# VictoriaMetrics/VictoriaMetrics

Hardware: NVIDIA H100
Metric: rollup samples/sec (block decode + rate, raw samples decoded and scanned per second) (higher is better)
Workload: dtype int64 codec -> f64 rollup

## Files before the change

victoriametrics_b200/csrc/api.cu:

```cuda
#include <cuda_runtime.h>
#include <cuda_fp16.h>
#include <stdarg.h>
#include <stdio.h>
#include <string.h>
#include <stdlib.h>

#include <algorithm>
#include <vector>

#include "common.cuh"
#include "decode.cu"
#include "rollup.cu"
#include "fused.cu"
#include "zstd.cu"
#include "marshal.inc"
#include "encode.cu"

static thread_local char g_err[512];
void vmb_set_error(const char* fmt, ...) {
    va_list ap;
    va_start(ap, fmt);
    vsnprintf(g_err, sizeof(g_err), fmt, ap);
    va_end(ap);
}
// ... 167 lines not shown
    vmb_ctx_comm_destroy(c);
    if (c->col_cache) vmb_series_free(c->col_cache);
    c->col_cache = nullptr;
    DevBuf* bufs[] = {&c->zscratch, &c->zlit, &c->zstatus, &c->zjobs, &c->zws, &c->args1, &c->args2, &c->rolled,
                      &c->counters, &c->tmp_out, &c->grp, &c->mheap, &c->mnext, &c->zseq, &c->bail, &c->sub_arrays, &c->fused_recs, &c->aggr_state, &c->grp_ids, &c->enc_vals, &c->enc_deltas, &c->enc_out, &c->enc_meta, &c->enc_frames,
                      &c->oa_keys, &c->oa_keys2, &c->oa_cell, &c->oa_meta, &c->cv_runs, &c->cv_aux, &c->cv_uniq};
    for (DevBuf* b : bufs) b->release();
    for (cudaEvent_t e : c->ev)
        if (e) cudaEventDestroy(e);
    for (cudaEvent_t e : c->zev) cudaEventDestroy(e);
    if (c->zstream) cudaStreamDestroy(c->zstream);
    if (c->h_pinned) cudaFreeHost(c->h_pinned);
    if (c->pipe && c->pipe_destroy) c->pipe_destroy(c->pipe);
    delete c;
}
extern "C" int vmb_ctx_set_stream(vmb_ctx* c, void* stream) {
    if (!c) return VMB_ERR_INVALID_ARG;
    c->stream = (cudaStream_t)stream;
    return VMB_OK;
}
extern "C" int vmb_ctx_set_dedup_interval(vmb_ctx* c, int64_t interval_ms) {
    if (!c || interval_ms < 0) return VMB_ERR_INVALID_ARG;
    c->dedup_interval = interval_ms;
    return VMB_OK;
}
extern "C" int vmb_ctx_set_fused(vmb_ctx* c, int enable) {
    if (!c) return VMB_ERR_INVALID_ARG;
    c->fused = enable != 0;
    return VMB_OK;
}
extern "C" int vmb_ctx_synchronize(vmb_ctx* c) {
    if (!c) return VMB_ERR_INVALID_ARG;
    CU(cudaSetDevice(c->device));
    CU(cudaStreamSynchronize(c->stream));
    return VMB_OK;
}
extern "C" uint64_t vmb_ctx_launch_count(const vmb_ctx* c) { return c ? c->launches : 0; }
extern "C" float vmb_ctx_last_stage_ms(const vmb_ctx* c, int stage) {
    return (c && stage >= 0 && stage < ST__COUNT) ? c->stage_ms[stage] : 0.f;
}
extern "C" int vmb_ctx_enable_stage_timing(vmb_ctx* c, int enable) {
    if (!c) return VMB_ERR_INVALID_ARG;
    c->timing = enable != 0;
    return VMB_OK;
}
extern "C" void* vmb_host_alloc(size_t bytes) {
    void* p = nullptr;
    if (cudaHostAlloc(&p, bytes ? bytes : 1, cudaHostAllocDefault) != cudaSuccess) return nullptr;
    return p;
}
extern "C" void vmb_host_free(void* p) {
    if (p) cudaFreeHost(p);
}

static inline uint64_t be_get(const uint8_t* s, int n) {
    uint64_t v = 0;
    for (int i = 0; i < n; i++) v = (v << 8) | s[i];
    return v;
}
extern "C" int vmb_block_desc_from_header(vmb_block_desc* d, const uint8_t h[81], uint8_t tsid_out[24]) {
    if (!d || !h) return VMB_ERR_INVALID_ARG;
    memset(d, 0, sizeof(*d));
    if (tsid_out) memcpy(tsid_out, h, 24);
    auto unzz = [](uint64_t u) { return (int64_t)(u >> 1) ^ -(int64_t)(u & 1); };
    d->min_ts = unzz(be_get(h + 24, 8));
    d->max_ts = unzz(be_get(h + 32, 8));
    d->first_value = unzz(be_get(h + 40, 8));
    d->ts_off = be_get(h + 48, 8);
    d->val_off = be_get(h + 56, 8);
    d->ts_size = (uint32_t)be_get(h + 64, 4);
    d->val_size = (uint32_t)be_get(h + 68, 4);
    d->rows = (uint32_t)be_get(h + 72, 4);
    uint16_t u = (uint16_t)be_get(h + 76, 2);
    d->scale = (int16_t)((int16_t)(u >> 1) ^ (int16_t)(-(int16_t)(u & 1)));
    d->ts_mt = h[78];
    d->val_mt = h[79];
    d->precision_bits = h[80];
    if (d->rows == 0 || d->rows > 16384) return VMB_ERR_ROWS;
    if (d->ts_mt > 6 || d->val_mt > 6) return VMB_ERR_MARSHAL_TYPE;
    if (d->precision_bits < 1 || d->precision_bits > 64) return VMB_ERR_INVALID_ARG;
    if (d->ts_size > 131072 || d->val_size > 131072) return VMB_ERR_INVALID_ARG;
    return VMB_OK;
}

static inline void be_put(uint8_t* d, uint64_t v, int n) {
    for (int i = 0; i < n; i++) d[i] = (uint8_t)(v >> (8 * (n - 1 - i)));
}
extern "C" int vmb_block_header_marshal(uint8_t h[81], const vmb_block_desc* d, const uint8_t tsid[24]) {
    if (!h || !d) return VMB_ERR_INVALID_ARG;
    if (tsid) memcpy(h, tsid, 24);
    else memset(h, 0, 24);
    auto zz = [](int64_t v) { return (uint64_t)((v << 1) ^ (v >> 63)); };
    be_put(h + 24, zz(d->min_ts), 8);
    be_put(h + 32, zz(d->max_ts), 8);
    be_put(h + 40, zz(d->first_value), 8);
    be_put(h + 48, d->ts_off, 8);
    be_put(h + 56, d->val_off, 8);
    be_put(h + 64, d->ts_size, 4);
    be_put(h + 68, d->val_size, 4);
    be_put(h + 72, d->rows, 4);
    be_put(h + 76, (uint16_t)((d->scale << 1) ^ (d->scale >> 15)), 2);
    h[78] = d->ts_mt;
    h[79] = d->val_mt;
    h[80] = d->precision_bits;
    return VMB_OK;
}
extern "C" int vmb_index_block_unmarshal(vmb_block_desc* out, uint8_t* tsids, size_t count, const uint8_t* data, size_t len) {
    if (!out || !data || count == 0) return VMB_ERR_INVALID_ARG;
    if (len != count * 81) {
        vmb_set_error("invalid number of block headers found: %zu bytes; want %zu block headers", len, count);
        return len % 81 ? VMB_ERR_SHORT_SRC : VMB_ERR_ROWS;
    }
    for (size_t i = 0; i < count; i++) {
        int rc = vmb_block_desc_from_header(&out[i], data + i * 81, tsids ? tsids + i * 24 : nullptr);
        if (rc) {
            vmb_set_error("cannot unmarshal block header %zu: error %d", i, rc);
            return rc;
        }
        if (i && memcmp(data + (i - 1) * 81, data + i * 81, 24) > 0) {
            vmb_set_error("block headers must be sorted by tsid (header %zu)", i);
            return VMB_ERR_INVALID_ARG;
        }
    }
    return VMB_OK;
}
extern "C" int vmb_metaindex_rows_unmarshal(vmb_metaindex_row* out, size_t cap, size_t* n_out, const uint8_t* data, size_t len) {
    if (!n_out || (len && !data)) return VMB_ERR_INVALID_ARG;
    *n_out = 0;
    if (len == 0) {
        vmb_set_error("expecting non-zero metaindex rows; got zero");
        return VMB_ERR_SHORT_SRC;
    }
    if (len % 56) {
        vmb_set_error("cannot unmarshal metaindexRow #%zu: %zu trailing bytes", len / 56, len % 56);
        return VMB_ERR_SHORT_SRC;
    }
    const size_t n = len / 56;
    *n_out = n;
    if (n > cap || !out) return VMB_ERR_CAP;
    auto unzz = [](uint64_t u) { return (int64_t)(u >> 1) ^ -(int64_t)(u & 1); };
    for (size_t i = 0; i < n; i++) {
        const uint8_t* r = data + i * 56;
        vmb_metaindex_row& m = out[i];
        memcpy(m.tsid, r, 24);
        m.block_headers_count = (uint32_t)be_get(r + 24, 4);
        m.min_ts = unzz(be_get(r + 28, 8));
        m.max_ts = unzz(be_get(r + 36, 8));
        m.index_block_offset = be_get(r + 44, 8);
        m.index_block_size = (uint32_t)be_get(r + 52, 4);
        if (m.block_headers_count == 0) {
            vmb_set_error("metaindexRow #%zu: BlockHeadersCount must be greater than 0", i);
            return VMB_ERR_ROWS;
        }
        if (m.index_block_size > 131072) {
            vmb_set_error("metaindexRow #%zu: too big IndexBlockSize %u", i, m.index_block_size);
            return VMB_ERR_INVALID_ARG;
        }
        if (i && memcmp(r - 56, r, 24) > 0) {
            vmb_set_error("metaindexRow values must be sorted by TSID (row %zu)", i);
            return VMB_ERR_INVALID_ARG;
        }
    }
    return VMB_OK;
}
extern "C" int vmb_metaindex_row_marshal(uint8_t out[56], const vmb_metaindex_row* m) {
    if (!out || !m) return VMB_ERR_INVALID_ARG;
    auto zz = [](int64_t v) { return (uint64_t)((v << 1) ^ (v >> 63)); };
    memcpy(out, m->tsid, 24);
    be_put(out + 24, m->block_headers_count, 4);
    be_put(out + 28, zz(m->min_ts), 8);
    be_put(out + 36, zz(m->max_ts), 8);
    be_put(out + 44, m->index_block_offset, 8);
    be_put(out + 52, m->index_block_size, 4);
    return VMB_OK;
}

template <class T>
static int dev_alloc(T** p, size_t n) {
    *p = nullptr;
    cudaError_t e = cudaMalloc((void**)p, (n ? n : 1) * sizeof(T));
    if (e != cudaSuccess) {
        vmb_set_error("cudaMalloc(%zu) failed: %s", n * sizeof(T), cudaGetErrorString(e));
        return VMB_ERR_NOMEM;
    }
    return 0;
}

extern "C" void vmb_blocks_free(vmb_blocks* b) {
    if (!b) return;
    if (b->ctx) cudaSetDevice(b->ctx->device);
    cudaFree(b->d_arrays);
    cudaFree(b->d_payload_alloc);
    delete b;
}
extern "C" size_t vmb_blocks_count(const vmb_blocks* b) { return b ? b->nblocks : 0; }
extern "C" uint64_t vmb_blocks_rows(const vmb_blocks* b) { return b ? b->rows : 0; }
extern "C" uint64_t vmb_blocks_compressed_bytes(const vmb_blocks* b) { return b ? b->compressed : 0; }

struct BlocksPlan {
    std::vector<ColInfo> cols;
    std::vector<uint64_t> row_off;
    std::vector<uint32_t> huf, gen, bad, ser_first, ser_nblocks, fused, unfused, huf_upto;
    std::vector<uint64_t> ser_merge_off;
    uint64_t rows = 0, compressed = 0, scratch_total = 0, merge_rows = 0, seq_total = 0;
    bool needs_lit = false;
    unsigned long long content_bound = 0;
};
static void plan_layout(BlocksPlan& pl, const vmb_block_desc* descs, size_t nblocks) {
    pl.row_off.resize(nblocks + 1);
    pl.rows = 0;
    pl.ser_first.clear();
    pl.ser_nblocks.clear();
    for (size_t b = 0; b < nblocks; b++) {
        const vmb_block_desc& d = descs[b];
        pl.row_off[b] = pl.rows;
        pl.rows += d.rows <= 16384 ? d.rows : 0;
        if (b == 0 || d.series_idx != descs[b - 1].series_idx) {
            pl.ser_first.push_back((uint32_t)b);
            pl.ser_nblocks.push_back(1);
        } else {
            pl.ser_nblocks.back()++;
        }
    }
    pl.row_off[nblocks] = pl.rows;
    pl.ser_merge_off.assign(pl.ser_first.size(), UINT64_MAX);
    pl.merge_rows = 0;
    std::vector<uint32_t> order;
    for (size_t s = 0; s < pl.ser_first.size(); s++) {
        const uint32_t fb = pl.ser_first[s], nb = pl.ser_nblocks[s];
        if (nb < 2) continue;
        order.resize(nb);
        for (uint32_t k = 0; k < nb; k++) order[k] = fb + k;
        std::stable_sort(order.begin(), order.end(), [&](uint32_t a, uint32_t b) { return descs[a].min_ts < descs[b].min_ts; });
        uint64_t r = pl.row_off[fb], total = 0;
        bool overlap = false;
        for (uint32_t k = 0; k < nb; k++) {
            const vmb_block_desc& d = descs[order[k]];
            const uint64_t rows = d.rows <= 16384 ? d.rows : 0;
            pl.row_off[order[k]] = r + total;
            total += rows;
            if (k + 1 < nb && d.max_ts >= descs[order[k + 1]].min_ts) overlap = true;
        }
        if (overlap) {
            pl.ser_merge_off[s] = pl.merge_rows;
            pl.merge_rows += total;
        }
    }
}

static int plan_blocks(BlocksPlan& pl, const vmb_block_desc* descs, size_t nblocks, const uint8_t* payload, size_t payload_len) {
    pl.cols.resize(2 * nblocks);
    uint64_t scratch = 0;
    for (size_t b = 0; b < nblocks; b++) {
        const vmb_block_desc& d = descs[b];
        pl.compressed += (uint64_t)d.ts_size + d.val_size;
        if ((uint64_t)d.ts_off + d.ts_size > payload_len || (uint64_t)d.val_off + d.val_size > payload_len) {
            vmb_set_error("block %zu: payload range outside the arena (len %zu)", b, payload_len);
            return VMB_ERR_INVALID_ARG;
        }
        for (int which = 0; which < 2; which++) {
            ColInfo& ci = pl.cols[2 * b + which];
            memset(&ci, 0, sizeof(ci));
            int mt = which ? d.val_mt : d.ts_mt;
            if (mt != 1 && mt != 4) continue;
            const uint8_t* src = payload + (which ? d.val_off : d.ts_off);
            uint32_t len = which ? d.val_size : d.ts_size;
            uint32_t cs = 0;
            bool needs_lit = false;
            uint32_t nseq = 0;
            ci.kind = zstd_classify_host(src, len, d.rows <= 16384 ? d.rows : 0, &cs, &needs_lit, &nseq, pl.content_bound);
            if (ci.kind == VMB_ZK_HUF && nseq) {
                if (pl.seq_total + nseq > 0xffffffffull) {
                    vmb_set_error("more than 2^32 zstd sequences in one batch: split it");
                    return VMB_ERR_INVALID_ARG;
                }
                ci.nseq = nseq;
                ci.seq_rec_off = (uint32_t)pl.seq_total;
                pl.seq_total += nseq;
            }
            ci.content_size = cs;
            uint32_t col = (uint32_t)(2 * b + which);
            if (ci.kind == VMB_ZK_BAD) {
                pl.bad.push_back(col);
                continue;
            }
            ci.scratch_off = scratch;
            scratch += ((uint64_t)cs + 15) & ~(uint64_t)15;
            if (needs_lit) pl.needs_lit = true;
            if (ci.kind == VMB_ZK_HUF) pl.huf.push_back(col);
            else pl.gen.push_back(col);
        }
    }
    pl.scratch_total = scratch;
    plan_layout(pl, descs, nblocks);
    for (size_t s = 0; s < pl.ser_first.size(); s++) {
        const uint32_t fb = pl.ser_first[s];
        const vmb_block_desc& d = descs[fb];
        const bool ok = pl.ser_nblocks[s] == 1 && d.ts_mt == 2 && d.precision_bits >= 64 && d.rows >= 2 && d.rows <= 16384 &&
                        d.val_mt >= 1 && d.val_mt <= 6 && pl.cols[2 * fb + 1].kind != VMB_ZK_BAD;
        (ok ? pl.fused : pl.unfused).push_back((uint32_t)s);
    }
    std::vector<uint32_t> fpos(2 * nblocks, UINT32_MAX);
    for (size_t j = 0; j < pl.fused.size(); j++) fpos[2 * (size_t)pl.ser_first[pl.fused[j]] + 1] = (uint32_t)j;
    std::stable_sort(pl.huf.begin(), pl.huf.end(), [&](uint32_t a, uint32_t b) {
        return fpos[a] + 1u < fpos[b] + 1u;
    });
    pl.huf_upto.assign(pl.fused.size() + 1, (uint32_t)pl.huf.size());
    for (size_t i = pl.huf.size(); i-- > 0;) {
        const uint32_t j = fpos[pl.huf[i]];
        if (j == UINT32_MAX) break;
        pl.huf_upto[j] = (uint32_t)i;
    }
    for (size_t j = pl.fused.size(); j-- > 0;) pl.huf_upto[j] = std::min(pl.huf_upto[j], pl.huf_upto[j + 1]);
    return 0;
}

struct PlanArrays {
    size_t nblocks, descs, cols, row_off, huf, gen, bad, ser_first, ser_nblocks, ser_merge_off, extra[3], bytes;
    PlanArrays(const BlocksPlan& pl, size_t nb, size_t n_extra0 = 0, size_t n_extra1 = 0, size_t n_extra2 = 0) : nblocks(nb) {
        const size_t ns = pl.ser_first.size();
        size_t o = 0;
        auto take = [&](size_t n) {
            const size_t at = o;
            o = al16(o + n);
            return at;
        };
        descs = take(nb * sizeof(vmb_block_desc));
        cols = take(2 * nb * sizeof(ColInfo));
        row_off = take((nb + 1) * sizeof(uint64_t));
        huf = take(pl.huf.size() * 4);
        gen = take(pl.gen.size() * 4);
        bad = take(pl.bad.size() * 4);
        ser_first = take(ns * 4);
        ser_nblocks = take(ns * 4);
        ser_merge_off = take(ns * 8);
        extra[0] = take(n_extra0 * 4);
        extra[1] = take(n_extra1 * 4);
        extra[2] = take(n_extra2 * 4);
        bytes = o;
    }
    void pack(uint8_t* h, const BlocksPlan& pl, const vmb_block_desc* d) const {
        auto put = [h](size_t at, const auto& v) {
            if (!v.empty()) memcpy(h + at, v.data(), v.size() * sizeof(v[0]));
        };
        if (d && nblocks) memcpy(h + descs, d, nblocks * sizeof(vmb_block_desc));
        put(cols, pl.cols);
        put(row_off, pl.row_off);
        put(huf, pl.huf);
        put(gen, pl.gen);
        put(bad, pl.bad);
        put(ser_first, pl.ser_first);
        put(ser_nblocks, pl.ser_nblocks);
        put(ser_merge_off, pl.ser_merge_off);
    }
    void bind(vmb_blocks* b, uint8_t* d, const BlocksPlan& pl) const {
        b->nblocks = nblocks;
        b->nseries = pl.ser_first.size();
        b->rows = pl.rows;
        b->compressed = pl.compressed;
        b->scratch_total = pl.scratch_total;
        b->merge_rows = pl.merge_rows;
        b->seq_total = pl.seq_total;
        b->needs_lit = pl.needs_lit;
        b->n_huf = (uint32_t)pl.huf.size();
        b->n_gen = (uint32_t)pl.gen.size();
        b->n_bad = (uint32_t)pl.bad.size();
        b->d_descs = (vmb_block_desc*)(d + descs);
        b->d_cols = (ColInfo*)(d + cols);
        b->d_row_off = (uint64_t*)(d + row_off);
        b->d_huf_list = (uint32_t*)(d + huf);
        b->d_gen_list = (uint32_t*)(d + gen);
        b->d_bad_list = (uint32_t*)(d + bad);
        b->d_ser_first = (uint32_t*)(d + ser_first);
        b->d_ser_nblocks = (uint32_t*)(d + ser_nblocks);
        b->d_ser_merge_off = (uint64_t*)(d + ser_merge_off);
    }
    uint32_t* extra_at(uint8_t* base, int i) const { return (uint32_t*)(base + extra[i]); }
};

static int blocks_upload_impl(vmb_ctx* ctx, const vmb_block_desc* descs, size_t nblocks, const uint8_t* payload, size_t payload_len,
                              vmb_blocks** out, unsigned long long content_bound) {
    if (!ctx || !out || (nblocks && !descs) || (payload_len && !payload) || nblocks > 0x7fffffffu / 2) return VMB_ERR_INVALID_ARG;
    CU(cudaSetDevice(ctx->device));
    BlocksPlan pl;
    pl.content_bound = content_bound;
    int rc = plan_blocks(pl, descs, nblocks, payload, payload_len);
    if (rc) return rc;
    const PlanArrays L(pl, nblocks, pl.fused.size());
    std::vector<uint8_t> h(L.bytes);
    L.pack(h.data(), pl, descs);
    if (!pl.fused.empty()) memcpy(L.extra_at(h.data(), 0), pl.fused.data(), pl.fused.size() * 4);
    vmb_blocks* b = new vmb_blocks();
    b->ctx = ctx;
    rc = dev_alloc(&b->d_arrays, L.bytes);
    if (!rc) rc = dev_alloc(&b->d_payload_alloc, payload_len + 128);
    if (!rc) {
        L.bind(b, b->d_arrays, pl);
        b->d_fused_list = L.extra_at(b->d_arrays, 0);
        b->d_payload = b->d_payload_alloc + 64;
        cudaStream_t st = ctx->stream;
        cudaError_t e = cudaMemcpyAsync(b->d_arrays, h.data(), L.bytes, cudaMemcpyHostToDevice, st);
        if (e == cudaSuccess) e = cudaMemsetAsync(b->d_payload_alloc, 0, 64, st);
        if (e == cudaSuccess && payload_len) e = cudaMemcpyAsync(b->d_payload, payload, payload_len, cudaMemcpyHostToDevice, st);
        if (e == cudaSuccess) e = cudaMemsetAsync(b->d_payload + payload_len, 0, 64, st);
        if (e == cudaSuccess) e = cudaStreamSynchronize(st);
        if (e != cudaSuccess) {
            vmb_set_error("uploading %zu blocks: %s", nblocks, cudaGetErrorString(e));
            rc = VMB_ERR_CUDA;
        }
    }
    if (rc) {
        vmb_blocks_free(b);
        return rc;
    }
    b->h_descs.assign(descs, descs + nblocks);
    b->h_cols = pl.cols;
    b->h_ser_first = pl.ser_first;
    b->h_ser_nblocks = pl.ser_nblocks;
    b->h_fused = pl.fused;
    b->h_unfused = pl.unfused;
    b->h_huf_upto = pl.huf_upto;
    *out = b;
    return VMB_OK;
}
extern "C" int vmb_blocks_upload(vmb_ctx* ctx, const vmb_block_desc* descs, size_t nblocks, const uint8_t* payload,
                                 size_t payload_len, vmb_blocks** out) {
    return blocks_upload_impl(ctx, descs, nblocks, payload, payload_len, out, 0);
}

extern "C" int vmb_blocks_upload_part(vmb_ctx* ctx, const uint8_t* headers, size_t nblocks, const uint8_t* timestamps_bin, size_t ts_len,
                                      const uint8_t* values_bin, size_t val_len, vmb_blocks** out) {
    if (!ctx || !out || (nblocks && !headers) || (ts_len && !timestamps_bin) || (val_len && !values_bin)) return VMB_ERR_INVALID_ARG;
    std::vector<vmb_block_desc> descs(nblocks);
    size_t total = 0;
    uint8_t prev_tsid[24], tsid[24];
    uint32_t series = 0;
    for (size_t i = 0; i < nblocks; i++) {
        vmb_block_desc& d = descs[i];
        int rc = vmb_block_desc_from_header(&d, headers + i * 81, tsid);
        if (rc) return rc;
        if (d.ts_off > ts_len || d.ts_size > ts_len - d.ts_off || d.val_off > val_len || d.val_size > val_len - d.val_off) {
            vmb_set_error("block %zu references bytes outside the part files (timestamps [%llu, +%u) of %zu, values [%llu, +%u) of %zu)", i,
                          (unsigned long long)d.ts_off, d.ts_size, ts_len, (unsigned long long)d.val_off, d.val_size, val_len);
            return VMB_ERR_SHORT_SRC;
        }
        if (i && memcmp(tsid, prev_tsid, 24) != 0) series++;
        memcpy(prev_tsid, tsid, 24);
        d.series_idx = series;
        total += al16((size_t)d.ts_size) + al16((size_t)d.val_size);
    }
    std::vector<uint8_t> arena(total + 16);
    size_t pos = 0;
    for (size_t i = 0; i < nblocks; i++) {
        vmb_block_desc& d = descs[i];
        if (d.ts_size) memcpy(arena.data() + pos, timestamps_bin + d.ts_off, d.ts_size);
        d.ts_off = pos;
        pos += al16((size_t)d.ts_size);
        if (d.val_size) memcpy(arena.data() + pos, values_bin + d.val_off, d.val_size);
        d.val_off = pos;
        pos += al16((size_t)d.val_size);
    }
    return blocks_upload_impl(ctx, descs.data(), nblocks, arena.data(), pos, out, 0);
}

extern "C" void vmb_series_free(vmb_series* s) {
    if (!s) return;
    if (s->ctx) cudaSetDevice(s->ctx->device);
    cudaFree(s->d_ts);
    cudaFree(s->d_vals);
    cudaFree(s->d_meta);
    cudaFree(s->d_blk_lo);
    cudaFree(s->d_blk_hi);
    cudaFree(s->d_blk_status);
    delete s;
}
extern "C" size_t vmb_series_count(const vmb_series* s) { return s ? s->nseries : 0; }
extern "C" uint64_t vmb_series_rows(const vmb_series* s) { return s ? s->rows : 0; }

__global__ void k_set_status(int32_t* status, const uint32_t* list, uint32_t n, int32_t v) {
    uint32_t i = blockIdx.x * blockDim.x + threadIdx.x;
    if (i < n) status[list[i]] = v;
}

static void zstd_huf_range(vmb_ctx* ctx, const vmb_blocks* b, ZstdParams Z, uint32_t h0, uint32_t h1, cudaStream_t st) {
    if (h0 >= h1) return;
    Z.jobs = (HufJob*)ctx->zjobs.p + h0;
    Z.list = b->d_huf_list + h0;
    Z.count = h1 - h0;
    launch_zstd_prepare(Z, st);
    launch_huf_decode(Z, ctx->huf_ctas_per_sm, st);
    count_launch(ctx, 2);
    if (b->needs_lit) {
        launch_zstd_sequences(Z, st);
        count_launch(ctx, 2);
    }
}

static int run_zstd(vmb_ctx* ctx, const vmb_blocks* b, int32_t** d_zstatus_out, uint32_t huf_end = UINT32_MAX,
                    ZstdParams* Zrest = nullptr) {
    cudaStream_t st = ctx->stream;
    *d_zstatus_out = nullptr;
    if (b->n_huf + b->n_gen + b->n_bad == 0) return VMB_OK;
    int rc;
    if ((rc = ctx->zscratch.reserve(b->scratch_total + 64))) return rc;
    if ((rc = ctx->zstatus.reserve(2 * b->nblocks * sizeof(int32_t)))) return rc;
    int32_t* d_zstatus = (int32_t*)ctx->zstatus.p;
    CU(cudaMemsetAsync(d_zstatus, 0, 2 * b->nblocks * sizeof(int32_t), st));
    if (b->needs_lit && (rc = ctx->zlit.reserve(b->scratch_total + 64))) return rc;
    ZstdParams Z;
    memset(&Z, 0, sizeof(Z));
    Z.descs = b->d_descs;
    Z.cols = b->d_cols;
    Z.payload = b->d_payload;
    Z.scratch = (uint8_t*)ctx->zscratch.p;
    Z.lit = b->needs_lit ? (uint8_t*)ctx->zlit.p : nullptr;
    if (b->seq_total) {
        if ((rc = ctx->zseq.reserve(b->seq_total * 8))) return rc;
        Z.seq_rec = (unsigned long long*)ctx->zseq.p;
    }
    Z.status = d_zstatus;
    if (b->n_bad) {
        k_set_status<<<(b->n_bad + 127) / 128, 128, 0, st>>>(d_zstatus, b->d_bad_list, b->n_bad, VMB_ERR_ZSTD);
        count_launch(ctx);
    }
    const uint32_t ws_threads = VMB_SMS * 2u * 32u;
    if (b->needs_lit || b->n_gen) {
        if ((rc = ctx->zws.reserve((size_t)ws_threads * zstd_serial_ws_bytes()))) return rc;
        Z.ws = ctx->zws.p;
        Z.ws_count = ws_threads;
    }
    if (b->n_huf && (rc = ctx->zjobs.reserve((size_t)b->n_huf * sizeof(HufJob)))) return rc;
    if (Zrest) *Zrest = Z;
    zstd_huf_range(ctx, b, Z, 0, std::min(huf_end, b->n_huf), st);
    if (b->n_gen) {
        Z.list = b->d_gen_list;
        Z.count = b->n_gen;
        launch_zstd_serial(Z, 1, st);
        count_launch(ctx);
    }
    *d_zstatus_out = d_zstatus;
    return VMB_OK;
}

static int run_decode(vmb_ctx* ctx, const vmb_blocks* b, vmb_series* s, int64_t tr_min, int64_t tr_max, uint32_t flags,
                      unsigned int* d_failed, bool zstd_done = false, int32_t* d_zstatus_in = nullptr,
                      const uint32_t* d_blk_map = nullptr, const ColInfo* d_zcols_in = nullptr) {
    cudaStream_t st = ctx->stream;
    if (ctx->timing && !zstd_done) CU(cudaEventRecord(ctx->ev[ST_ZSTD], st));
    int32_t* d_zstatus = d_zstatus_in;
    if (!zstd_done) {
        int rc = run_zstd(ctx, b, &d_zstatus);
        if (rc) return rc;
    }
    if (ctx->timing && !zstd_done) CU(cudaEventRecord(ctx->ev[ST_DECODE], st));
    DecodeParams D;
    memset(&D, 0, sizeof(D));
    D.descs = b->d_descs;
    D.cols = b->d_cols;
    D.payload = b->d_payload;
    D.scratch = (const uint8_t*)ctx->zscratch.p;
    D.zstd_status = d_zstatus;
    D.zstd_cols = zstd_done ? d_zcols_in : b->d_cols;
    D.blk_map = d_blk_map;
    D.row_off = b->d_row_off;
    D.ts_out = s->d_ts;
    D.val_out = s->d_vals;
    D.blk_lo = s->d_blk_lo;
    D.blk_hi = s->d_blk_hi;
    D.status = s->d_blk_status;
    D.nblocks = (uint32_t)b->nblocks;
    D.flags = flags;
    D.tr_min = tr_min;
    D.tr_max = tr_max;
    launch_decode_columns(D, st);
    count_launch(ctx);
    RollupParams R;
    memset(&R, 0, sizeof(R));
    R.meta = s->d_meta;
    R.nseries = (uint32_t)s->nseries;
    R.ser_first_block = b->d_ser_first;
    R.ser_nblocks = b->d_ser_nblocks;
    R.row_off = b->d_row_off;
    R.blk_lo = s->d_blk_lo;
    R.blk_hi = s->d_blk_hi;
    R.descs = b->d_descs;
    R.blk_status = s->d_blk_status;
    R.failed_blocks = d_failed;
    R.ser_merge_off = b->d_ser_merge_off;
    R.rows_total = b->rows;
    R.ts = s->d_ts;
    R.vals = s->d_vals;
    R.dedup_interval = (flags & VMB_DECODE_VALUES_AS_INT64) ? 0 : ctx->dedup_interval;
    launch_series_assemble(R, st);
    count_launch(ctx);
    if (b->merge_rows) {
        if (flags & VMB_DECODE_VALUES_AS_INT64) {
            vmb_set_error("series with overlapping blocks cannot be assembled from VMB_DECODE_VALUES_AS_INT64 columns");
            return VMB_ERR_INVALID_ARG;
        }
        int rc;
        if ((rc = ctx->mheap.reserve(b->nblocks * sizeof(uint32_t)))) return rc;
        if ((rc = ctx->mnext.reserve(b->nblocks * sizeof(uint32_t)))) return rc;
        R.merge_heap = (uint32_t*)ctx->mheap.p;
        R.merge_next = (uint32_t*)ctx->mnext.p;
        launch_series_merge(R, st);
        count_launch(ctx);
    }
    if (R.dedup_interval > 0) {
        launch_series_dedup(R, st);
        count_launch(ctx);
    }
    if (ctx->timing && !zstd_done) CU(cudaEventRecord(ctx->ev[ST_PREAMBLE], st));
    CU(cudaGetLastError());
    return 0;
}
// ... 570 lines not shown
}
static int group_csr(const uint32_t* group_ids, const uint32_t* sub, size_t n, uint32_t ngroups, uint32_t* start, uint32_t* order) {
    memset(start, 0, ((size_t)ngroups + 1) * 4);
    for (size_t i = 0; i < n; i++) {
        const size_t s = sub ? sub[i] : i;
        if (group_ids[s] >= ngroups) return group_id_error(group_ids[s], s, ngroups);
        start[group_ids[s] + 1]++;
    }
    for (uint32_t g = 0; g < ngroups; g++) start[g + 1] += start[g];
    std::vector<uint32_t> cur(start, start + ngroups);
    for (size_t i = 0; i < n; i++) order[cur[group_ids[sub ? sub[i] : i]]++] = (uint32_t)i;
    return 0;
}
static int upload_group_csr(vmb_ctx* ctx, std::vector<uint32_t>& h, const uint32_t* group_ids, const uint32_t* sub, size_t n,
                            uint32_t ngroups, size_t extra, uint32_t** d_csr) {
    h.resize((size_t)ngroups + 1 + n);
    int rc = group_csr(group_ids, sub, n, ngroups, h.data(), h.data() + ngroups + 1);
    if (!rc) rc = ctx->grp.reserve((h.size() + extra) * sizeof(uint32_t));
    if (rc) return rc;
    *d_csr = (uint32_t*)ctx->grp.p;
    CU(cudaMemcpyAsync(*d_csr, h.data(), h.size() * 4, cudaMemcpyHostToDevice, ctx->stream));
    return 0;
}

struct AggrTarget {
    int aggr_id;
    const uint32_t* group_ids;
    uint32_t ngroups;
    double* d_values;
    double* d_counts;
};
static void launch_aggr_merge(vmb_ctx* ctx, cudaStream_t st, int aggr_id, double* dv, double* dc, const double* sv, const double* sc,
                              size_t n) {
    k_aggr_merge<<<(unsigned)((n + 255) / 256), 256, 0, st>>>(aggr_id, dv, dc, sv, sc, n);
    count_launch(ctx);
}
static void aggr_fold(vmb_ctx* ctx, cudaStream_t st, const AggrTarget& t, const double* rolled, const uint32_t* d_csr, int64_t points,
                      double* d_partial) {
    const size_t cells = (size_t)t.ngroups * (size_t)points;
    AggrParams A;
    A.rolled = rolled;
    A.grp_start = d_csr;
    A.grp_series = d_csr + t.ngroups + 1;
    A.values = d_partial ? d_partial : t.d_values;
    A.counts = d_partial ? d_partial + cells : t.d_counts;
    A.ngroups = t.ngroups;
    A.npoints = (uint32_t)points;
    A.aggr = t.aggr_id;
    k_aggr_fold<<<(unsigned)((cells + 127) / 128), 128, 0, st>>>(A);
    count_launch(ctx);
    if (d_partial) launch_aggr_merge(ctx, st, t.aggr_id, t.d_values, t.d_counts, A.values, A.counts, cells);
}

extern "C" int vmb_rollup_aggr_partial(vmb_ctx* ctx, vmb_series* s, const vmb_rollup_cfg* cfg, int aggr_id,
                                       const uint32_t* group_ids, uint32_t ngroups, double* d_values, double* d_counts,
                                       double* d_rollup_scratch, uint64_t* samples_scanned) {
    if (!ctx || !s || !group_ids || !d_values || !d_counts || ngroups == 0 || aggr_id < 0 || aggr_id > VMB_AGGR_GROUP)
        return VMB_ERR_INVALID_ARG;
    int64_t points;
    int rc = check_cfg(cfg, &points);
    if (rc) return rc;
    CU(cudaSetDevice(ctx->device));
    cudaStream_t st = ctx->stream;
    size_t total = (size_t)s->nseries * (size_t)points;
    double* d_rolled = d_rollup_scratch;
    if (!d_rolled) {
        if ((rc = ctx->rolled.reserve(total * 8))) return rc;
        d_rolled = (double*)ctx->rolled.p;
    }
    const AggrTarget t = {aggr_id, group_ids, ngroups, d_values, d_counts};
    std::vector<uint32_t> h_csr;
    uint32_t* d_csr;
    if ((rc = upload_group_csr(ctx, h_csr, group_ids, nullptr, s->nseries, ngroups, 0, &d_csr))) return rc;
    Counters c;
    if ((rc = counters_zero(ctx, st, &c))) return rc;
    if (ctx->timing) CU(cudaEventRecord(ctx->ev[ST_PREAMBLE], st));
    if ((rc = run_rollup(ctx, s, cfg, points, d_rolled, c.d_scanned))) return rc;
    aggr_fold(ctx, st, t, d_rolled, d_csr, points, nullptr);
    if (ctx->timing) CU(cudaEventRecord(ctx->ev[ST_FUSED], st));
    if ((rc = counters_read(ctx, st, samples_scanned))) return rc;
    collect_stage_times(ctx, ST_PREAMBLE, ST_FUSED);
    return VMB_OK;
}

extern "C" int vmb_aggr_merge(vmb_ctx* ctx, int aggr_id, double* dv, double* dc, const double* sv, const double* sc, size_t n) {
    if (!ctx || !dv || !dc || !sv || !sc) return VMB_ERR_INVALID_ARG;
    CU(cudaSetDevice(ctx->device));
    if (n) launch_aggr_merge(ctx, ctx->stream, aggr_id, dv, dc, sv, sc, n);
    CU(cudaGetLastError());
    return VMB_OK;
}
extern "C" int vmb_aggr_prepare_allreduce(vmb_ctx* ctx, int aggr_id, double* dv, const double* dc, size_t n) {
    if (!ctx || !dv || !dc) return VMB_ERR_INVALID_ARG;
    CU(cudaSetDevice(ctx->device));
    if (n) {
        k_aggr_prepare_allreduce<<<(unsigned)((n + 255) / 256), 256, 0, ctx->stream>>>(aggr_id, dv, dc, n);
        count_launch(ctx);
    }
    CU(cudaGetLastError());
    return VMB_OK;
}
extern "C" int vmb_aggr_finalize(vmb_ctx* ctx, int aggr_id, double* dv, const double* dc, size_t n, double* out_host) {
    if (!ctx || !dv || !dc) return VMB_ERR_INVALID_ARG;
    CU(cudaSetDevice(ctx->device));
    if (n) {
        k_aggr_finalize<<<(unsigned)((n + 255) / 256), 256, 0, ctx->stream>>>(aggr_id, dv, dc, n);
        count_launch(ctx);
        if (out_host) CU(cudaMemcpyAsync(out_host, dv, n * 8, cudaMemcpyDeviceToHost, ctx->stream));
    }
    CU(cudaStreamSynchronize(ctx->stream));
    return VMB_OK;
}

static int column_cache_view(vmb_ctx* ctx, const vmb_blocks* b, vmb_series* view) {
    vmb_series* c = ctx->col_cache;
    if (c && (c->rows < b->rows + b->merge_rows || c->nseries < b->nseries || c->nblocks < b->nblocks)) {
        vmb_series_free(c);
        ctx->col_cache = c = nullptr;
    }
    if (!c) {
        int rc = alloc_series_for(ctx, b, &c);
        if (rc) return rc;
        ctx->col_cache = c;
    }
    *view = *c;
    view->nseries = b->nseries;
    view->nblocks = b->nblocks;
    view->rows = b->rows + b->merge_rows;
    view->stale_dropped = view->resets_removed = view->rolled = false;
    view->pre_applied = 0;
    return 0;
}

static const size_t FUSED_SMEM = (sizeof(FusedSmem) + 15) & ~(size_t)15;
template <typename K>
static uint32_t fused_grid(K kernel) {
    int blocks_per_sm = 0;
    cudaFuncSetAttribute(kernel, cudaFuncAttributeMaxDynamicSharedMemorySize, (int)FUSED_SMEM);
    if (cudaOccupancyMaxActiveBlocksPerMultiprocessor(&blocks_per_sm, kernel, FU_THREADS, FUSED_SMEM) != cudaSuccess || blocks_per_sm < 1)
        blocks_per_sm = 1;
    if (blocks_per_sm > FU_CTAS_PER_SM) blocks_per_sm = FU_CTAS_PER_SM;
    return VMB_SMS * (uint32_t)blocks_per_sm;
}

extern "C" int vmb_fused_grid(void) {
    static const uint32_t grid = fused_grid(k_fused_rollup<VMB_RF_RATE>);
    return (int)grid;
}
extern "C" int vmb_fused_grid_chunked(void) {
    return (int)std::min<uint32_t>((uint32_t)vmb_fused_grid(), VMB_SMS * FU_CTAS_PER_SM_OVERLAP);
}

static uint32_t fused_chunks(const vmb_ctx* ctx, const vmb_blocks* b) {
    const size_t nf = b->h_fused.size();
    uint32_t C = ctx->fused_chunks ? ctx->fused_chunks : FUSED_CHUNKS_DEFAULT;
    if (C > nf) C = (uint32_t)nf;
    if (C <= 1 || b->n_huf == 0) return 1;
    return b->h_huf_upto[nf / C] < b->n_huf ? C : 1u;
}

static uint32_t fused_ctas_per_sm(const vmb_ctx* ctx, uint32_t C, const vmb_rollup_cfg* cfg) {
    if (ctx->fused_ctas_per_sm) return ctx->fused_ctas_per_sm;
    (void)C;
    (void)cfg;
    return FU_CTAS_PER_SM;
}

static void launch_fused(const FusedParams& P, uint32_t ctas_per_sm, cudaStream_t st) {
    if (!P.nlist) return;
    const size_t smem0 = FUSED_SMEM;
#define FUSED_LAUNCH(KERNEL, SMEM)                                                                                \
    do {                                                                                                          \
        static const uint32_t grid0 = fused_grid(KERNEL);                                                         \
        uint32_t grid = std::min(grid0, VMB_SMS * ctas_per_sm);                                                   \
        if (grid > P.nlist) grid = P.nlist;                                                                       \
        KERNEL<<<grid, FU_THREADS, (SMEM), st>>>(P);                                                              \
    } while (0)
    switch (P.cfg.func_id) {
#define FUSED_CASE(F) case F: FUSED_LAUNCH((k_fused_rollup<F>), smem0); break;
        FUSED_CASE(VMB_RF_RATE)
        FUSED_CASE(VMB_RF_DELTA)
        FUSED_CASE(VMB_RF_AVG)
        FUSED_CASE(VMB_RF_MIN)
        FUSED_CASE(VMB_RF_MAX)
        FUSED_CASE(VMB_RF_SUM)
        FUSED_CASE(VMB_RF_COUNT)
        FUSED_CASE(VMB_RF_QUANTILE)
        FUSED_CASE(VMB_RF_DEFAULT_ROLLUP)
        FUSED_CASE(VMB_RF_IDERIV)
        FUSED_CASE(VMB_RF_IDELTA)
        FUSED_CASE(VMB_RF_LAST)
        FUSED_CASE(VMB_RF_FIRST)
        FUSED_CASE(VMB_RF_STDDEV)
        FUSED_CASE(VMB_RF_STDVAR)
        FUSED_CASE(VMB_RF_CHANGES)
        FUSED_CASE(VMB_RF_DERIV)
#undef FUSED_CASE
        default: FUSED_LAUNCH((k_fused_rollup<-1>), smem0); break;
    }
#undef FUSED_LAUNCH
}

static bool fused_enabled(const vmb_ctx* ctx, const vmb_blocks* b, const vmb_rollup_cfg* cfg) {
    return ctx->fused && !b->h_fused.empty() && ctx->dedup_interval == 0 && !(cfg->flags & VMB_RC_PRE_MASK);
}

static int run_unfused_subset(vmb_ctx* ctx, const vmb_blocks* b, const std::vector<uint32_t>& sub, int32_t* d_zstatus,
                              int64_t tr_min, int64_t tr_max, const vmb_rollup_cfg* cfg, int64_t points, double* d_out,
                              const Counters& c, bool dense_rows) {
    cudaStream_t st = ctx->stream;
    std::vector<vmb_block_desc> descs;
    std::vector<uint32_t> blk_map;
    BlocksPlan pl;
    for (size_t i = 0; i < sub.size(); i++) {
        const uint32_t fb = b->h_ser_first[sub[i]], nb = b->h_ser_nblocks[sub[i]];
        for (uint32_t k = 0; k < nb; k++) {
            vmb_block_desc d = b->h_descs[fb + k];
            d.series_idx = (uint32_t)i;
            descs.push_back(d);
            pl.cols.push_back(b->h_cols[2 * (size_t)(fb + k)]);
            pl.cols.push_back(b->h_cols[2 * (size_t)(fb + k) + 1]);
            blk_map.push_back(fb + k);
        }
    }
    const size_t cn = descs.size(), cs = sub.size();
    plan_layout(pl, descs.data(), cn);
    const PlanArrays L(pl, cn, cn, cs);
    std::vector<uint8_t> hs(L.bytes);
    L.pack(hs.data(), pl, descs.data());
    memcpy(L.extra_at(hs.data(), 0), blk_map.data(), cn * 4);
    memcpy(L.extra_at(hs.data(), 1), sub.data(), cs * 4);
    int rc;
    if ((rc = ctx->sub_arrays.reserve(L.bytes + 64))) return rc;
    CU(cudaMemcpyAsync(ctx->sub_arrays.p, hs.data(), L.bytes, cudaMemcpyHostToDevice, st));
    uint8_t* da = (uint8_t*)ctx->sub_arrays.p;
    vmb_blocks bv;
    bv.ctx = ctx;
    L.bind(&bv, da, pl);
    bv.d_payload = b->d_payload;
    vmb_series view;
    if ((rc = column_cache_view(ctx, &bv, &view))) return rc;
    rc = run_decode(ctx, &bv, &view, tr_min, tr_max, 0, c.d_failed, true, d_zstatus, L.extra_at(da, 0), b->d_cols);
    if (!rc) rc = run_rollup(ctx, &view, cfg, points, d_out, c.d_scanned, dense_rows ? nullptr : L.extra_at(da, 1), false);
    cudaError_t e = cudaStreamSynchronize(st);
    if (!rc && e != cudaSuccess) {
        vmb_set_error("un-fused sub-batch: %s", cudaGetErrorString(e));
        rc = VMB_ERR_CUDA;
    }
    return rc;
}

static bool aggr_fusable(int aggr_id) {
    return aggr_id == VMB_AGGR_SUM || aggr_id == VMB_AGGR_AVG || aggr_id == VMB_AGGR_COUNT || aggr_id == VMB_AGGR_GROUP ||
           aggr_id == VMB_AGGR_SUM2 || aggr_id == VMB_AGGR_MIN || aggr_id == VMB_AGGR_MAX;
}
__global__ void k_aggr_init(int aggr, double* dv, double* dc, size_t n) {
    size_t i = (size_t)blockIdx.x * blockDim.x + threadIdx.x;
    if (i >= n) return;
    dv[i] = aggr == VMB_AGGR_MIN ? D_INF : (aggr == VMB_AGGR_MAX ? -D_INF : 0.0);
    dc[i] = 0.0;
}

static int eval_fused(vmb_ctx* ctx, const vmb_blocks* b, int64_t tr_min, int64_t tr_max, const vmb_rollup_cfg* cfg, int64_t points,
                      double* d_out, const Counters& c, const AggrTarget* af) {
    cudaStream_t st = ctx->stream;
    int rc;
    if (af) {
        if ((rc = ctx->grp_ids.reserve((b->nseries + 1) * sizeof(uint32_t)))) return rc;
        CU(cudaMemcpyAsync(ctx->grp_ids.p, af->group_ids, b->nseries * sizeof(uint32_t), cudaMemcpyHostToDevice, st));
        const size_t cells = (size_t)af->ngroups * (size_t)points;
        k_aggr_init<<<(unsigned)((cells + 255) / 256), 256, 0, st>>>(af->aggr_id, af->d_values, af->d_counts, cells);
        count_launch(ctx);
    }
    const size_t nf = b->h_fused.size();
    if ((rc = ctx->bail.reserve((nf + 2) * sizeof(uint32_t)))) return rc;
    if ((rc = ctx->fused_recs.reserve(nf * sizeof(FuSeries)))) return rc;
    unsigned int* d_bail_count = (unsigned int*)ctx->bail.p;
    uint32_t* d_bail_list = (uint32_t*)ctx->bail.p + 2;
    FusedParams F;
    memset(&F, 0, sizeof(F));
    if ((rc = upload_cfg_args(ctx, cfg, points, &F.cfg))) return rc;
    F.descs = b->d_descs;
    F.cols = b->d_cols;
    F.payload = b->d_payload;
    F.ser_first_block = b->d_ser_first;
    F.out = d_out;
    if (af) {
        if ((rc = ctx->tmp_out.reserve((size_t)VMB_SMS * FU_CTAS_PER_SM * (size_t)points * 8))) return rc;
        F.out = (double*)ctx->tmp_out.p;
        F.aggr_values = af->d_values;
        F.aggr_counts = af->d_counts;
        F.group_ids = (const uint32_t*)ctx->grp_ids.p;
        F.aggr_id = af->aggr_id;
    }
    F.scanned = c.d_scanned;
    F.bail_list = d_bail_list;
    F.bail_count = d_bail_count;
    F.claim = d_bail_count + 1;
    F.npoints = (uint32_t)points;
    F.tr_min = tr_min;
    F.tr_max = tr_max;
    const uint32_t C = fused_chunks(ctx, b);
    auto chunk_begin = [&](uint32_t k) { return (uint32_t)(nf * k / C); };
    if (C > 1) {
        if (!ctx->zstream) CU(cudaStreamCreateWithFlags(&ctx->zstream, cudaStreamNonBlocking));
        while (ctx->zev.size() < C) {
            cudaEvent_t e;
            CU(cudaEventCreateWithFlags(&e, cudaEventDisableTiming));
            ctx->zev.push_back(e);
        }
    }
    if (ctx->timing) CU(cudaEventRecord(ctx->ev[ST_ZSTD], st));
    int32_t* d_zstatus = nullptr;
    ZstdParams Z = {};
    if ((rc = run_zstd(ctx, b, &d_zstatus, C > 1 ? b->h_huf_upto[chunk_begin(1)] : UINT32_MAX, &Z))) return rc;
    if (ctx->timing) CU(cudaEventRecord(ctx->ev[ST_DECODE], st));
    struct Join {
        cudaStream_t st;
        cudaEvent_t done = nullptr;
        ~Join() {
            if (done) cudaStreamWaitEvent(st, done, 0);
        }
    } join{st};
    if (C > 1) {
        CU(cudaEventRecord(ctx->zev[0], st));
        CU(cudaStreamWaitEvent(ctx->zstream, ctx->zev[0], 0));
        for (uint32_t k = 1; k < C; k++) {
            zstd_huf_range(ctx, b, Z, b->h_huf_upto[chunk_begin(k)], b->h_huf_upto[chunk_begin(k + 1)], ctx->zstream);
            cudaError_t e = cudaEventRecord(ctx->zev[k], ctx->zstream);
            if (e == cudaSuccess) join.done = ctx->zev[k];
            CU(e);
        }
    }
    CU(cudaMemsetAsync(d_bail_count, 0, 8, st));
    F.scratch = (const uint8_t*)ctx->zscratch.p;
    F.zstd_status = d_zstatus;
    const uint32_t ctas_per_sm = fused_ctas_per_sm(ctx, C, cfg);
    for (uint32_t k = 0; k < C; k++) {
        if (k) CU(cudaStreamWaitEvent(st, ctx->zev[k], 0));
        F.ser_list = b->d_fused_list + chunk_begin(k);
        F.nlist = chunk_begin(k + 1) - chunk_begin(k);
        FuSeries* recs = (FuSeries*)ctx->fused_recs.p + chunk_begin(k);
        F.recs = recs;
        if (F.nlist) {
            k_fused_series_records<<<(F.nlist + 127) / 128, 128, 0, st>>>(F, recs);
            count_launch(ctx);
        }
        launch_fused(F, ctas_per_sm, st);
        count_launch(ctx);
    }
    if (ctx->timing) CU(cudaEventRecord(ctx->ev[ST_PREAMBLE], st));
    CU(cudaGetLastError());
    unsigned int* h_bail = (unsigned int*)((char*)ctx->h_pinned + PIN_BAIL);
    CU(cudaMemcpyAsync(h_bail, d_bail_count, 4, cudaMemcpyDeviceToHost, st));
    CU(cudaStreamSynchronize(st));
    std::vector<uint32_t> sub(b->h_unfused);
    if (*h_bail) {
        const size_t n0 = sub.size();
        sub.resize(n0 + *h_bail);
        CU(cudaMemcpyAsync(sub.data() + n0, d_bail_list, (size_t)*h_bail * 4, cudaMemcpyDeviceToHost, st));
        CU(cudaStreamSynchronize(st));
        std::sort(sub.begin(), sub.end());
    }
    if (ctx->timing) {
        for (float& ms : ctx->stage_ms) ms = 0.f;
        stage_span(ctx, ST_ZSTD, ST_ZSTD, ST_DECODE);
        stage_span(ctx, ST_FUSED, ST_DECODE, ST_PREAMBLE);
    }
    if (!sub.empty()) {
        if (ctx->timing) CU(cudaEventRecord(ctx->ev[ST_ROLLUP], st));
        if (!af) {
            if ((rc = run_unfused_subset(ctx, b, sub, d_zstatus, tr_min, tr_max, cfg, points, d_out, c, false))) return rc;
        } else {
            const size_t cs = sub.size(), cells = (size_t)af->ngroups * (size_t)points;
            if ((rc = ctx->rolled.reserve((cs * (size_t)points + 2 * cells) * 8 + 64))) return rc;
            double* d_rows = (double*)ctx->rolled.p;
            if ((rc = run_unfused_subset(ctx, b, sub, d_zstatus, tr_min, tr_max, cfg, points, d_rows, c, true))) return rc;
            std::vector<uint32_t> h_csr;
            uint32_t* d_csr;
            if ((rc = upload_group_csr(ctx, h_csr, af->group_ids, sub.data(), cs, af->ngroups, 0, &d_csr))) return rc;
            aggr_fold(ctx, st, *af, d_rows, d_csr, points, d_rows + cs * (size_t)points);
            CU(cudaStreamSynchronize(st));
        }
        if (ctx->timing) {
            CU(cudaEventRecord(ctx->ev[ST_AGGR], st));
            CU(cudaStreamSynchronize(st));
            stage_span(ctx, ST_DECODE, ST_ROLLUP, ST_AGGR);
        }
    }
    return 0;
}

static int eval_device(vmb_ctx* ctx, const vmb_blocks* b, int64_t tr_min, int64_t tr_max, const vmb_rollup_cfg* cfg, int64_t points,
                       double* d_out, const AggrTarget* aggr, uint64_t* samples_scanned) {
    cudaStream_t st = ctx->stream;
    const bool fused = fused_enabled(ctx, b, cfg) && (!aggr || aggr_fusable(aggr->aggr_id));
    int rc;
    std::vector<uint32_t> h_csr;
    uint32_t* d_csr = nullptr;
    if (aggr && fused) {
        for (size_t i = 0; i < b->nseries; i++)
            if (aggr->group_ids[i] >= aggr->ngroups) return group_id_error(aggr->group_ids[i], i, aggr->ngroups);
    } else if (aggr) {
        if ((rc = upload_group_csr(ctx, h_csr, aggr->group_ids, nullptr, b->nseries, aggr->ngroups, 0, &d_csr))) return rc;
    }
    Counters c;
    if ((rc = counters_zero(ctx, st, &c))) return rc;
    if (fused) {
        if ((rc = eval_fused(ctx, b, tr_min, tr_max, cfg, points, d_out, c, aggr))) return rc;
        return counters_read(ctx, st, samples_scanned);
    }
    vmb_series view;
    if ((rc = column_cache_view(ctx, b, &view))) return rc;
    if ((rc = run_decode(ctx, b, &view, tr_min, tr_max, 0, c.d_failed))) return rc;
    double* d_rows = d_out;
    if (aggr) {
        if ((rc = ctx->rolled.reserve((size_t)b->nseries * (size_t)points * 8))) return rc;
        d_rows = (double*)ctx->rolled.p;
    }
    if ((rc = run_rollup(ctx, &view, cfg, points, d_rows, c.d_scanned))) return rc;
    if (aggr) {
        aggr_fold(ctx, st, *aggr, d_rows, d_csr, points, nullptr);
        if (ctx->timing) CU(cudaEventRecord(ctx->ev[ST_FUSED], st));
    }
    rc = counters_read(ctx, st, samples_scanned);
    if (rc && rc != VMB_ERR_BLOCK_FAILED) return rc;
    if (aggr) {
        collect_stage_times(ctx, ST_PREAMBLE, ST_FUSED);
    } else if (ctx->timing) {
        collect_stage_times(ctx, ST_ZSTD, ST_AGGR);
        ctx->stage_ms[ST_FUSED] = 0.f;
    }
    return rc;
}

extern "C" int vmb_eval_rollup_device(vmb_ctx* ctx, const vmb_blocks* b, int64_t tr_min, int64_t tr_max,
                                      const vmb_rollup_cfg* cfg, double* d_out, uint64_t* samples_scanned) {
    if (!ctx || !b || !d_out) return VMB_ERR_INVALID_ARG;
    int64_t points;
    int rc = check_cfg(cfg, &points);
    if (rc) return rc;
    CU(cudaSetDevice(ctx->device));
    return eval_device(ctx, b, tr_min, tr_max, cfg, points, d_out, nullptr, samples_scanned);
}

extern "C" int vmb_eval_rollup_aggr_device(vmb_ctx* ctx, const vmb_blocks* b, int64_t tr_min, int64_t tr_max,
                                           const vmb_rollup_cfg* cfg, int aggr_id, const uint32_t* group_ids, uint32_t ngroups,
                                           double* d_values, double* d_counts, uint64_t* samples_scanned) {
    if (!ctx || !b || !group_ids || !d_values || !d_counts || ngroups == 0 || aggr_id < 0 || aggr_id > VMB_AGGR_GROUP)
        return VMB_ERR_INVALID_ARG;
    int64_t points;
    int rc = check_cfg(cfg, &points);
    if (rc) return rc;
    CU(cudaSetDevice(ctx->device));
    const AggrTarget t = {aggr_id, group_ids, ngroups, d_values, d_counts};
    return eval_device(ctx, b, tr_min, tr_max, cfg, points, nullptr, &t, samples_scanned);
}

#include "pipeline.inc"
#include "topk.inc"
#include "comm.inc"
#include "matrix_ops.inc"
#include "aggr_matrix.inc"
#include "aggr_order.inc"
#include "transform.inc"
#include "range_transform.inc"
#include "histogram.inc"
#include "vmrange.inc"
#include "rank_aggr.inc"
#include "count_values.inc"
#include "vm_histogram.inc"
#include "rowset.inc"

#include <atomic>
#include <thread>
extern "C" int vmb_marshal_columns(uint8_t* dst, size_t cap, uint64_t* offs, uint8_t* mts, int64_t* firsts,
                                   const int64_t* vals, size_t ncols, size_t rows, uint8_t precision_bits, int nthreads) {
    if (!dst || !offs || !mts || !firsts || !vals || rows == 0) return VMB_ERR_INVALID_ARG;
    std::vector<std::vector<uint8_t>> outs(ncols);
    std::atomic<size_t> next{0};
    std::atomic<int> err{0};
    auto worker = [&]() {
        for (;;) {
            size_t c = next.fetch_add(1);
            if (c >= ncols) break;
            int mt = 0;
            int64_t first = 0;
            int rc = vmb_host::marshal_int64_array(outs[c], &mt, &first, vals + c * rows, rows, precision_bits);
            if (rc) err = rc;
            mts[c] = (uint8_t)mt;
            firsts[c] = first;
        }
    };
    if (nthreads <= 1) worker();
    else {
        std::vector<std::thread> th;
        for (int t = 0; t < nthreads; t++) th.emplace_back(worker);
        for (auto& t : th) t.join();
    }
    if (err.load()) return err.load();
    uint64_t o = 0;
    for (size_t c = 0; c < ncols; c++) {
        offs[c] = o;
        if (o + outs[c].size() > cap) return VMB_ERR_CAP;
        if (!outs[c].empty()) memcpy(dst + o, outs[c].data(), outs[c].size());
        o += outs[c].size();
    }
    offs[ncols] = o;
    return VMB_OK;
}

static int marshal_columns_dev(vmb_ctx* ctx, MarshalParams& M, uint64_t* offs, uint8_t* mts, int64_t* firsts, bool skip_mid,
                               const uint64_t** d_offs) {
    cudaStream_t st = ctx->stream;
    const size_t ncols = M.ncols;
    int rc;
    const size_t o_sizes = 0, o_mts = al16(o_sizes + ncols * 4), o_firsts = al16(o_mts + ncols), o_offs = al16(o_firsts + ncols * 8),
                 o_slot = o_offs + ncols * 8, o_zlen = o_slot + ncols * 8, o_flen = al16(o_zlen + ncols * 4),
                 o_csrc = al16(o_flen + ncols * 4), o_clen = al16(o_csrc + ncols * 8), o_out = al16(o_clen + ncols * 4);
    if ((rc = ctx->enc_meta.reserve(al16(o_out + (ncols + 1) * 8) + 64))) return rc;
    uint8_t* dm = (uint8_t*)ctx->enc_meta.p;
    M.sizes = (uint32_t*)(dm + o_sizes);
    M.mts = dm + o_mts;
    M.firsts = (int64_t*)(dm + o_firsts);
    M.offs = (const uint64_t*)(dm + o_offs);
    launch_marshal_plan(M, st);
    count_launch(ctx);
    std::vector<uint32_t> sizes(ncols);
    std::vector<uint8_t> pmts(ncols);
    CU(cudaMemcpyAsync(sizes.data(), M.sizes, ncols * 4, cudaMemcpyDeviceToHost, st));
    CU(cudaMemcpyAsync(pmts.data(), M.mts, ncols, cudaMemcpyDeviceToHost, st));
    CU(cudaMemcpyAsync(firsts, M.firsts, ncols * 8, cudaMemcpyDeviceToHost, st));
    CU(cudaStreamSynchronize(st));
    std::vector<uint8_t> up(o_flen - o_offs);
    uint64_t* soffs = (uint64_t*)up.data();
    uint64_t* slot = (uint64_t*)(up.data() + (o_slot - o_offs));
    uint32_t* zlen = (uint32_t*)(up.data() + (o_zlen - o_offs));
    uint64_t total = 0;
    for (size_t c = 0; c < ncols; c++) {
        soffs[c] = total;
        total += sizes[c];
    }
    const size_t min_compressible = 128;
    uint64_t so = al16(total);
    for (size_t c = 0; c < ncols; c++) {
        zlen[c] = (pmts[c] == 1 || pmts[c] == 4) && sizes[c] >= min_compressible ? sizes[c] : 0;
        if (skip_mid && zlen[c] > zw::kMaxBlock && zlen[c] < 262144u) zlen[c] = 0;
        slot[c] = so;
        so += zlen[c] ? al16(zw::raw_frame_len(zlen[c], 9)) : 0;
    }
    if ((rc = ctx->enc_out.reserve(so + 64))) return rc;
    if ((rc = ctx->enc_frames.reserve(total + 64))) return rc;
    CU(cudaMemcpyAsync(dm + o_offs, up.data(), up.size(), cudaMemcpyHostToDevice, st));
    M.out = (uint8_t*)ctx->enc_out.p;
    launch_marshal_pack(M, st);
    ZstdFrameJobs J;
    J.base = (uint8_t*)ctx->enc_out.p;
    J.src_off = (const uint64_t*)(dm + o_offs);
    J.len = (const uint32_t*)(dm + o_zlen);
    J.slot_off = (const uint64_t*)(dm + o_slot);
    J.frame_len = (uint32_t*)(dm + o_flen);
    J.n = (uint32_t)ncols;
    launch_zstd_frames(J, st);
    uint64_t* d_csrc = (uint64_t*)(dm + o_csrc);
    uint32_t* d_clen = (uint32_t*)(dm + o_clen);
    uint64_t* d_out = (uint64_t*)(dm + o_out);
    launch_marshal_select(M.sizes, J.src_off, J, M.mts, d_csrc, d_clen, (uint32_t)ncols, st);
    launch_scan_lens(d_clen, d_out, (uint32_t)ncols, st);
    launch_compact(J.base, d_csrc, d_out, (uint8_t*)ctx->enc_frames.p, (uint32_t)ncols, st);
    count_launch(ctx, 5);
    CU(cudaMemcpyAsync(offs, d_out, (ncols + 1) * 8, cudaMemcpyDeviceToHost, st));
    CU(cudaMemcpyAsync(mts, M.mts, ncols, cudaMemcpyDeviceToHost, st));
    CU(cudaStreamSynchronize(st));
    CU(cudaGetLastError());
    if (d_offs) *d_offs = d_out;
    return VMB_OK;
}

extern "C" int vmb_marshal_columns_gpu(vmb_ctx* ctx, uint8_t* dst, size_t cap, uint64_t* offs, uint8_t* mts, int64_t* firsts,
                                       const int64_t* vals, size_t ncols, size_t rows, uint8_t precision_bits, int nthreads) {
    if (!ctx || !dst || !offs || !mts || !firsts || !vals || rows == 0 || rows > 16384 || ncols > 0x7fffffffu || precision_bits < 1 ||
        precision_bits > 64)
        return VMB_ERR_INVALID_ARG;
    CU(cudaSetDevice(ctx->device));
    cudaStream_t st = ctx->stream;
    if (ncols == 0) {
        offs[0] = 0;
        return VMB_OK;
    }
    int rc;
    const size_t nvals = ncols * rows;
    if ((rc = ctx->enc_vals.reserve(nvals * 8))) return rc;
    const bool may_be_lossy = precision_bits < 64;
    if (may_be_lossy && (rc = ctx->enc_deltas.reserve(nvals * 8))) return rc;
    CU(cudaMemcpyAsync(ctx->enc_vals.p, vals, nvals * 8, cudaMemcpyHostToDevice, st));
    MarshalParams M;
    memset(&M, 0, sizeof(M));
    M.vals = (const int64_t*)ctx->enc_vals.p;
    M.deltas = may_be_lossy ? (int64_t*)ctx->enc_deltas.p : nullptr;
    M.ncols = (uint32_t)ncols;
    M.rows = (uint32_t)rows;
    M.pb = precision_bits;
    if ((rc = marshal_columns_dev(ctx, M, offs, mts, firsts, false, nullptr))) return rc;
    if (offs[ncols] > cap) return VMB_ERR_CAP;
    if (offs[ncols]) {
        CU(cudaMemcpyAsync(dst, ctx->enc_frames.p, offs[ncols], cudaMemcpyDeviceToHost, st));
        CU(cudaStreamSynchronize(st));
    }
    return VMB_OK;
}

extern "C" int vmb_float_to_decimal_columns(vmb_ctx* ctx, int64_t* dst, int16_t* scales, const double* src, size_t ncols, size_t rows) {
    if (!ctx || !dst || !scales || !src || rows == 0 || ncols > 0x7fffffffu || rows > 0x7fffffffu) return VMB_ERR_INVALID_ARG;
    if (ncols == 0) return VMB_OK;
    CU(cudaSetDevice(ctx->device));
    cudaStream_t st = ctx->stream;
    const size_t n = ncols * rows;
    int rc;
    if ((rc = ctx->enc_vals.reserve(n * 8))) return rc;
    if ((rc = ctx->enc_deltas.reserve(n * 8))) return rc;
    if ((rc = ctx->enc_meta.reserve(al16(n * 2) + al16(ncols * 2) + 64))) return rc;
    double* d_src = (double*)ctx->enc_vals.p;
    int64_t* d_dst = (int64_t*)ctx->enc_deltas.p;
    int16_t* d_ea = (int16_t*)ctx->enc_meta.p;
    int16_t* d_sc = (int16_t*)((uint8_t*)ctx->enc_meta.p + al16(n * 2));
    CU(cudaMemcpyAsync(d_src, src, n * 8, cudaMemcpyHostToDevice, st));
// ... 13 lines not shown
```

Baseline: 74.84 billion.

## Split Huffman zstd columns by sequence need and overlap phases across two streams

Huffman-compressed columns are now sorted so that literal-only columns feeding fused series come last. When the fused rollup runs as a single chunk, the zstd work is split into two ranges. The prepare step for the literal-only range runs on a side stream while the other range is prepared and Huffman-decoded on the main stream. Sequence execution for the first range then overlaps the literal-only range's Huffman decode. The aim is to hide zstd prepare and sequence latency behind independent decode work, at the cost of extra launches and event synchronisation.

```diff
diff --git a/victoriametrics_b200/csrc/api.cu b/victoriametrics_b200/csrc/api.cu
--- a/victoriametrics_b200/csrc/api.cu
+++ b/victoriametrics_b200/csrc/api.cu
@@ -493,15 +493,12 @@
     }
     std::vector<uint32_t> fpos(2 * nblocks, UINT32_MAX);
     for (size_t j = 0; j < pl.fused.size(); j++) fpos[2 * (size_t)pl.ser_first[pl.fused[j]] + 1] = (uint32_t)j;
+    auto lit_only = [&](uint32_t col) { return fpos[col] != UINT32_MAX && pl.cols[col].nseq == 0; };
     std::stable_sort(pl.huf.begin(), pl.huf.end(), [&](uint32_t a, uint32_t b) {
-        return fpos[a] + 1u < fpos[b] + 1u;
+        return ((uint64_t)lit_only(a) << 32 | (uint32_t)(fpos[a] + 1u)) < ((uint64_t)lit_only(b) << 32 | (uint32_t)(fpos[b] + 1u));
     });
     pl.huf_upto.assign(pl.fused.size() + 1, (uint32_t)pl.huf.size());
-    for (size_t i = pl.huf.size(); i-- > 0;) {
-        const uint32_t j = fpos[pl.huf[i]];
-        if (j == UINT32_MAX) break;
-        pl.huf_upto[j] = (uint32_t)i;
-    }
+    for (size_t i = pl.huf.size(); i-- > 0 && lit_only(pl.huf[i]);) pl.huf_upto[fpos[pl.huf[i]]] = (uint32_t)i;
     for (size_t j = pl.fused.size(); j-- > 0;) pl.huf_upto[j] = std::min(pl.huf_upto[j], pl.huf_upto[j + 1]);
     return 0;
 }
@@ -1678,9 +1675,11 @@
     F.tr_max = tr_max;
     const uint32_t C = fused_chunks(ctx, b);
     auto chunk_begin = [&](uint32_t k) { return (uint32_t)(nf * k / C); };
-    if (C > 1) {
+    const uint32_t mid = b->h_huf_upto[0];
+    const bool split = C == 1 && mid < b->n_huf;
+    if (C > 1 || split) {
         if (!ctx->zstream) CU(cudaStreamCreateWithFlags(&ctx->zstream, cudaStreamNonBlocking));
-        while (ctx->zev.size() < C) {
+        while (ctx->zev.size() < std::max(C, 4u)) {
             cudaEvent_t e;
             CU(cudaEventCreateWithFlags(&e, cudaEventDisableTiming));
             ctx->zev.push_back(e);
@@ -1689,8 +1688,7 @@
     if (ctx->timing) CU(cudaEventRecord(ctx->ev[ST_ZSTD], st));
     int32_t* d_zstatus = nullptr;
     ZstdParams Z = {};
-    if ((rc = run_zstd(ctx, b, &d_zstatus, C > 1 ? b->h_huf_upto[chunk_begin(1)] : UINT32_MAX, &Z))) return rc;
-    if (ctx->timing) CU(cudaEventRecord(ctx->ev[ST_DECODE], st));
+    if ((rc = run_zstd(ctx, b, &d_zstatus, C > 1 ? b->h_huf_upto[chunk_begin(1)] : (split ? 0u : UINT32_MAX), &Z))) return rc;
     struct Join {
         cudaStream_t st;
         cudaEvent_t done = nullptr;
@@ -1698,6 +1696,40 @@
             if (done) cudaStreamWaitEvent(st, done, 0);
         }
     } join{st};
+    if (split) {
+        auto range = [&](uint32_t h0, uint32_t h1) {
+            ZstdParams R = Z;
+            R.jobs = (HufJob*)ctx->zjobs.p + h0;
+            R.list = b->d_huf_list + h0;
+            R.count = h1 - h0;
+            return R;
+        };
+        const ZstdParams Zs = range(0, mid), Zl = range(mid, b->n_huf);
+        cudaStream_t zs = ctx->zstream;
+        CU(cudaEventRecord(ctx->zev[0], st));
+        CU(cudaStreamWaitEvent(zs, ctx->zev[0], 0));
+        launch_zstd_prepare(Zl, zs);
+        cudaError_t e = cudaEventRecord(ctx->zev[1], zs);
+        if (e == cudaSuccess) join.done = ctx->zev[1];
+        CU(e);
+        launch_zstd_prepare(Zs, st);
+        launch_huf_decode(Zs, ctx->huf_ctas_per_sm, st);
+        count_launch(ctx, 3);
+        CU(cudaEventRecord(ctx->zev[2], st));
+        CU(cudaStreamWaitEvent(st, ctx->zev[1], 0));
+        launch_huf_decode(Zl, ctx->huf_ctas_per_sm, st);
+        count_launch(ctx);
+        if (b->needs_lit) {
+            CU(cudaStreamWaitEvent(zs, ctx->zev[2], 0));
+            launch_zstd_sequences(Zs, zs);
+            count_launch(ctx, 2);
+        }
+        e = cudaEventRecord(ctx->zev[3], zs);
+        if (e == cudaSuccess) join.done = ctx->zev[3];
+        CU(e);
+        CU(cudaStreamWaitEvent(st, ctx->zev[3], 0));
+    }
+    if (ctx->timing) CU(cudaEventRecord(ctx->ev[ST_DECODE], st));
     if (C > 1) {
         CU(cudaEventRecord(ctx->zev[0], st));
         CU(cudaStreamWaitEvent(ctx->zstream, ctx->zev[0], 0));
```

Result: slower. 73.05 billion, median of 6 (-2.4%).
